# iden3/circom

Measured on NVIDIA B200. Metric: witnesses/s, higher is better.
Workload: dtype u256 (8x u32 limbs, Montgomery)

## Files before the change

circom_b200/csrc/capi.cu:

```cuda
#include <cuda_runtime.h>
#include <dlfcn.h>
#include <emmintrin.h>
#include <nccl.h>

#include <cstdio>
#include <cstdlib>
#include <algorithm>
#include <chrono>
#include <condition_variable>
#include <cstring>
#include <functional>
#include <map>
#include <memory>
#include <mutex>
#include <thread>
#include <stdexcept>
#include <string>
#include <vector>

#include "../../include/circom_b200.h"
#include "kernels.cuh"
#include "tape_calls.h"
#include "tape.h"
#include "hostpack.h"
// ... 195 lines not shown
        out = it->second;
        return CW_OK;
    }
    const Tape &t = c->tape;
    DevTape d;
    int rc;
    if ((rc = upload(&d.ops, t.ops.data(), t.ops.size() * 4))) return rc;
    if ((rc = upload(&d.items, t.items.data(), t.items.size() * 4))) return rc;
    {
        std::vector<uint32_t> heads(t.n_items() * 4);
        for (size_t k = 0; k < t.n_items(); ++k) memcpy(&heads[k * 4], &t.ops[(size_t)t.items[k] * 4], 16);
        if ((rc = upload(&d.heads, heads.data(), heads.size() * 4))) return rc;
    }
    if ((rc = upload(&d.level_start, t.level_start.data(), t.level_start.size() * 4))) return rc;
    {
        std::vector<uint32_t> info(t.n_levels(), 0);
        for (size_t l = 0; l < t.n_levels(); ++l) {
            bool tail = true;
            for (uint32_t k = t.level_start[l + 1]; k-- > t.level_start[l];) {
                const uint32_t opc = t.ops[(size_t)t.items[k] * 4] & 0xFFu;
                const bool single = t.items[k + 1] - t.items[k] == 1;
                const bool is_call = opc == 45u && single;
                if (opc == 45u && !(single && tail)) return fail(CW_ESTATE, "internal: a call is not at the end of its level");
                if (is_call) ++info[l];
                else tail = false;
                for (uint32_t w = t.items[k]; w < t.items[k + 1]; ++w) {
                    const uint32_t o = t.ops[(size_t)w * 4] & 0xFFu;
                    if (o == 28u || o == 5u) {
                        if (!single) return fail(CW_ESTATE, "internal: a fused work item contains INV / POW");
                        info[l] |= 0x80000000u;
                        d.has_slow = true;
                    }
                }
            }
        }
        if ((rc = upload(&d.level_info, info.data(), info.size() * 4))) return rc;
    }
    if ((rc = upload(&d.consts, t.consts.data(), t.consts.size() * 32))) return rc;
    if ((rc = upload(&d.input_slot, t.input_slot.data(), t.input_slot.size() * 4))) return rc;
    if ((rc = upload(&d.fn_code, t.fn_code.data(), t.fn_code.size() * 4))) return rc;
    if ((rc = upload(&d.fn_info, t.fn_info.data(), t.fn_info.size() * 4))) return rc;
    if ((rc = upload(&d.call_tab, t.call_tab.data(), t.call_tab.size() * 4))) return rc;
    if ((rc = upload(&d.wloc, t.witness_slot.data(), t.witness_slot.size() * 4))) return rc;
    if ((rc = upload(&d.pk_bit, L.bit_loc.data(), L.bit_loc.size() * 4))) return rc;
    if ((rc = upload(&d.pk_u64, L.u64_loc.data(), L.u64_loc.size() * 4))) return rc;
    if ((rc = upload(&d.pk_full, L.full_loc.data(), L.full_loc.size() * 4))) return rc;
    c->dev[device] = d;
    out = d;
    return CW_OK;
}

template <int PR, bool CALLS, bool BP, int BT, bool FU>
static void launch_tape_k(const TapeDev &tp, cw_batch *b, u32 tiles, u32 th) {
    tape_exec_kernel<PR, CALLS, BP, BT, FU><<<tiles, th, 0, b->stream>>>(tp, b->slots, b->plane, b->bt_log2, b->first_assert_d,
                                                                         b->err_d, b->batch);
}
template <int PR>
static void launch_tape(const TapeDev &tp, cw_batch *b, u32 tiles, u32 th, bool calls, bool bp, bool fused) {
    if (calls) {
        launch_tape_calls(PR, tp, b->slots, b->plane, b->bt_log2, b->first_assert_d, b->err_d, b->batch, tiles, th, bp, fused,
                          b->stream);
    } else if (fused) {
        if (b->bt_log2 == 5) launch_tape_k<PR, false, true, 5, true>(tp, b, tiles, th);
        else launch_tape_k<PR, false, true, -1, true>(tp, b, tiles, th);
    } else if (bp) {
        if (b->bt_log2 == 0) launch_tape_k<PR, false, true, 0, false>(tp, b, tiles, th);
        else if (b->bt_log2 == 5) launch_tape_k<PR, false, true, 5, false>(tp, b, tiles, th);
        else launch_tape_k<PR, false, true, -1, false>(tp, b, tiles, th);
    } else {
        if (b->bt_log2 == 0) launch_tape_k<PR, false, false, 0, false>(tp, b, tiles, th);
        else launch_tape_k<PR, false, false, -1, false>(tp, b, tiles, th);
    }
}

extern "C" {

int cw_version(void) { return 100; }
const char *cw_last_error(void) { return g_err.c_str(); }
int cw_device_count(void) {
    int n = 0;
    if (cudaGetDeviceCount(&n) != cudaSuccess) {
        cudaGetLastError();
        return 0;
    }
    return n;
}

int cw_circuit_load_mem(const void *data, size_t len, uint32_t flags, cw_circuit **out) {
    if (!data || !out) return fail(CW_EINVAL, "null argument");
    cw_circuit *c = new cw_circuit();
    try {
        lower_circuit((const uint8_t *)data, len, flags, c->tape);
    } catch (const std::exception &e) {
        delete c;
        return fail(CW_EFORMAT, e.what());
    }
    *out = c;
    return CW_OK;
}

int cw_circuit_load(const char *path, uint32_t flags, cw_circuit **out) {
    if (!path || !out) return fail(CW_EINVAL, "null argument");
    FILE *f = fopen(path, "rb");
    if (!f) return fail(CW_EIO, std::string("cannot open ") + path);
    fseek(f, 0, SEEK_END);
    long sz = ftell(f);
    fseek(f, 0, SEEK_SET);
    std::vector<uint8_t> buf(sz);
// ... 1518 lines not shown
```

circom_b200/csrc/flatten.cpp:

```cpp
#include <algorithm>
#include <bitset>
#include <cstdio>
#include <cstring>
#include <functional>
#include <stdexcept>
#include <unordered_map>

#include "../../include/circom_b200.h"
#include "tape.h"

namespace cw {

uint64_t fnv1a(const char *s, size_t n) {
    uint64_t h = 0xCBF29CE484222325ULL;
    for (size_t i = 0; i < n; ++i) {
        h ^= (uint64_t)(int64_t)(signed char)s[i];
        h *= 0x100000001B3ULL;
    }
    return h;
}

namespace {

enum { K_NONE = 0, K_OWN = 1, K_SUB = 2, K_CONST = 3, K_TMP = 4, K_ONE = 5 };
// ... 9 lines not shown
};
struct Tmpl {
    std::string name;
    uint32_t n_out, n_in, n_inter, n_tmp, n_own;
    std::vector<uint32_t> subs;
    std::vector<IrOp> ops;
    std::vector<uint32_t> lc_len;
    std::vector<Term> terms;
    std::vector<uint8_t> tmp_zero_only;
    uint64_t total_signals = 0, total_components = 0;
};

inline int rk(uint64_t r) { return (int)(r >> 56); }
inline uint32_t rsub(uint64_t r) { return (uint32_t)((r >> 32) & 0xFFFFFF); }
inline uint32_t ridx(uint64_t r) { return (uint32_t)r; }

struct Reader {
    const uint8_t *p, *end;
    template <class T>
    T get() {
        if (p + sizeof(T) > end) throw std::runtime_error("cb2c: truncated");
        T v;
        memcpy(&v, p, sizeof(T));
        p += sizeof(T);
        return v;
    }
    const uint8_t *bytes(size_t n) {
        if (n > (size_t)(end - p)) throw std::runtime_error("cb2c: truncated");
        const uint8_t *r = p;
        p += n;
        return r;
    }
    size_t left() const { return (size_t)(end - p); }
    void expect(uint64_t count, uint64_t bytes_each) const {
        if (count * bytes_each > left()) throw std::runtime_error("cb2c: truncated (count exceeds the file)");
    }
    std::string str() {
        uint32_t n = get<uint32_t>();
        const uint8_t *b = bytes((size_t)(((uint64_t)n + 3) & ~3ull));
        return std::string((const char *)b, n);
    }
};

struct Val {
    uint32_t slot[3] = {NO_SLOT, NO_SLOT, NO_SLOT};
    int32_t cid = -1;
    uint16_t bits = 256;
    uint8_t org_op = 0;
    int32_t org_a = -1, org_b = -1;
    int32_t fld_src = -1, bf_src = -1;
    uint16_t fld_k = 0, fld_m = 0, bf_lo = 0, bf_len = 0;
};

enum { DOP_BITS = 29, DOP_ASSERT_BOOL = 30, DOP_MULSMALL = 31, DOP_BITSIP = 32, DOP_ASSERT_FITS = 33 };
inline bool c_is_immediate(uint32_t opcode) {
    return opcode == CW_OP_ASSERT || opcode == CW_OP_ASSERT_EQ || opcode == DOP_BITS || opcode == DOP_ASSERT_BOOL ||
           opcode == DOP_BITSIP || opcode == DOP_ASSERT_FITS;
}
inline bool is_assert_op(uint32_t opcode) {
    return opcode == CW_OP_ASSERT || opcode == CW_OP_ASSERT_EQ || opcode == DOP_ASSERT_BOOL || opcode == DOP_ASSERT_FITS;
}

inline size_t n_live_ops(const std::vector<uint8_t> &live, uint32_t n_pre, size_t n_prov) {
    size_t n = 0;
    for (size_t i = 0; i < n_prov; ++i) n += live[n_pre + i];
    return n;
}
inline int subtree_need(uint32_t i, const std::vector<uint32_t> &kid_a, const std::vector<uint32_t> &kid_b) {
    const uint32_t a = kid_a[i], b = kid_b[i];
    if (a == NO_SLOT && b == NO_SLOT) return 1;
    if (a == NO_SLOT) return subtree_need(b, kid_a, kid_b);
    if (b == NO_SLOT) return subtree_need(a, kid_a, kid_b);
    const int na = subtree_need(a, kid_a, kid_b), nb = subtree_need(b, kid_a, kid_b);
    return std::max(std::max(na, nb), std::min(na, nb) + 1);
}

static uint32_t coalesce_function_copies(uint32_t *code, uint32_t n_instr, uint32_t n_regs, const std::vector<uint32_t> &fn_params) {
    constexpr uint32_t MAXR = 192;
    if (n_regs > MAXR || n_instr < 2) return n_instr;
    using Set = std::bitset<MAXR>;
    enum { JMP = 40, JZ = 41, RET = 42, LOADX = 43, STOREX = 44, CALLF = 45, COPY = 24 };
    auto is_reg = [&](uint32_t o) { return !(o & 0xC0000000u) && o < n_regs; };
    Set pinned;
    std::vector<uint8_t> target(n_instr + 1, 0);
    for (uint32_t i = 0; i < n_instr; ++i) {
        const uint32_t *w = &code[5 * (size_t)i];
        uint32_t lo = 0, hi = 0;
        if (w[0] == LOADX) { lo = w[2] & 0x3FFFFFFFu; hi = w[4] & 0x3FFFFFFFu; }
        else if (w[0] == STOREX) { lo = w[2] & 0x3FFFFFFFu; hi = w[1] & 0x3FFFFFFFu; }
        else if (w[0] == RET && (w[3] & 0x3FFFFFFFu) > 1) { lo = w[2]; hi = lo + (w[3] & 0x3FFFFFFFu); }
        else if (w[0] == CALLF) {
            for (uint32_t r = w[3]; r < w[3] + fn_params[w[2] & 0x3FFFFFFFu] && r < n_regs; ++r) pinned.set(r);
            if ((w[4] & 0x3FFFFFFFu) > 1) { lo = w[1]; hi = lo + (w[4] & 0x3FFFFFFFu); }
        }
        for (uint32_t r = lo; r < hi && r < n_regs; ++r) pinned.set(r);
        if (w[0] == JMP) target[std::min(w[2] & 0x3FFFFFFFu, n_instr)] = 1;
        if (w[0] == JZ) target[std::min(w[3] & 0x3FFFFFFFu, n_instr)] = 1;
    }
    std::vector<Set> use(n_instr), live_in(n_instr), live_out(n_instr);
    std::vector<int> def(n_instr, -1);
    auto add_use = [&](uint32_t i, uint32_t o) { if (is_reg(o) && !pinned.test(o)) use[i].set(o); };
    for (uint32_t i = 0; i < n_instr; ++i) {
        const uint32_t *w = &code[5 * (size_t)i];
        switch (w[0]) {
            case JMP: break;
            case JZ: add_use(i, w[2]); break;
            case RET: if ((w[3] & 0x3FFFFFFFu) <= 1) add_use(i, w[2]); break;
// ... 1149 lines not shown
            std::unordered_map<int32_t, uint32_t> entry_of_value;
            for (uint64_t i = 0; i < W; ++i) entry_of_value.emplace(sig_vid[T.witness2signal[i]], (uint32_t)i);
            std::unordered_map<std::string, uint32_t> const_at;
            auto log_const = [&](const U256 &v) {
                std::string key((const char *)v.v, 32);
                auto it = const_at.find(key);
                if (it != const_at.end()) return it->second;
                T.log_consts.push_back(v);
                return const_at.emplace(std::move(key), (uint32_t)T.log_consts.size() - 1).first->second;
            };
            for (const PendingLog &pl : pending_logs) {
                Tape::LogArg a;
                a.kind = pl.kind;
                a.last = pl.last ? 1 : 0;
                a.idx = (uint32_t)pl.idx;
                if (pl.kind == 2) a.idx = log_const(ir_consts[pl.idx]);
                if (pl.kind == 1) {
                    const int32_t v = sig_vid[pl.idx];
                    auto it = entry_of_value.find(v);
                    if (it != entry_of_value.end()) a.idx = it->second;
                    else if (vals[v].cid >= 0) { a.kind = 2; a.idx = log_const(ir_consts[vals[v].cid]); }
                    else throw std::runtime_error("lowering: log() of a signal whose value is not part of the witness");
                }
                T.log_args.push_back(a);
            }
        }
        std::vector<int64_t> claimed;
        std::vector<uint32_t> wsrc(W);
        auto grow = [&]() { claimed.resize(n_pre + pops.size() / 4, -1); };
        grow();
        for (uint64_t i = 0; i < W; ++i) {
            int32_t v = sig_vid[T.witness2signal[i]];
            uint32_t src;
            if (vals[v].cid >= 0) src = emit(CW_OP_COPY, const_operand(vals[v].cid, FC));
            else src = need(v, FC);
            grow();
            if (claimed[src] >= 0) {
                src = emit(CW_OP_COPY, src);
                grow();
            }
            claimed[src] = (int64_t)i;
            wsrc[i] = src;
            uint32_t wb = vbits(v);
            T.wit_bits.push_back((uint16_t)std::min<uint32_t>(wb, 256));
            if (wb <= 1) { T.pk_bit_wire.push_back((uint32_t)i); T.wit_class.push_back(0); }
            else if (wb <= 64) { T.pk_u64_wire.push_back((uint32_t)i); T.wit_class.push_back(1); }
            else { T.pk_full_wire.push_back((uint32_t)i); T.wit_class.push_back(2); }
        }
        size_t n_prov = pops.size() / 4;
        std::vector<uint16_t> slot_bits(n_pre + n_prov, 256);
        for (const Val &v : vals)
            if (v.cid < 0 && v.slot[FC] != NO_SLOT && v.slot[FC] < slot_bits.size())
                slot_bits[v.slot[FC]] = std::min<uint16_t>(slot_bits[v.slot[FC]], v.bits);
        for (uint64_t i = 0; i < W; ++i) {
            uint32_t wb = vbits(sig_vid[T.witness2signal[i]]);
            slot_bits[wsrc[i]] = std::min<uint16_t>(slot_bits[wsrc[i]], (uint16_t)wb);
        }
        std::vector<uint8_t> live(n_pre + n_prov, 0);
        for (uint64_t i = 0; i < W; ++i) live[wsrc[i]] = 1;
        for (size_t i = n_prov; i-- > 0;) {
            uint32_t *o = &pops[i * 4];
            bool is_assert = is_assert_op(o[0]);
            if (!is_assert && !live[n_pre + i]) continue;
            live[n_pre + i] = 1;
            if (o[0] == 45) {
                uint32_t n = pcalls[o[1] + 1];
                for (uint32_t k = 0; k < n; ++k) {
                    uint32_t a = pcalls[o[1] + 2 + k];
                    if (!(a & OPERAND_CONST)) live[a] = 1;
                }
                continue;
            }
            for (int k = 1; k <= 3; ++k) {
                if (k == 3 && c_is_immediate(o[0])) break;
                if (o[k] != NO_SLOT && !(o[k] & OPERAND_CONST)) live[o[k]] = 1;
            }
        }
        constexpr uint32_t FUSE_MAX = 24;
        std::vector<uint8_t> fusedf(n_prov, 0);
        std::vector<uint32_t> kid_a(n_prov, NO_SLOT), kid_b(n_prov, NO_SLOT);
        {
            std::vector<uint32_t> uses(n_pre + n_prov, 0), cons(n_pre + n_prov, NO_SLOT);
            std::vector<uint8_t> cons_pos(n_pre + n_prov, 0);
            for (size_t i = 0; i < n_prov; ++i) {
                if (!live[n_pre + i]) continue;
                const uint32_t *o = &pops[i * 4];
                if (o[0] == 45) {
                    uint32_t n = pcalls[o[1] + 1];
                    for (uint32_t k = 0; k < n; ++k) {
                        uint32_t x = pcalls[o[1] + 2 + k];
                        if (!(x & OPERAND_CONST)) uses[x] += 2;
                    }
                    continue;
                }
                for (int k = 1; k <= 3; ++k) {
                    if (k == 3 && c_is_immediate(o[0])) break;
                    if (o[k] == NO_SLOT || (o[k] & OPERAND_CONST)) continue;
                    ++uses[o[k]];
                    cons[o[k]] = (uint32_t)i;
                    cons_pos[o[k]] = (uint8_t)k;
                }
            }
            std::vector<uint8_t> need(n_prov, 1);
            std::vector<uint32_t> gsize(n_prov, 1);
            const bool fuse_on = (flags & CW_FLAG_FUSE) && !(flags & CW_FLAG_NO_PEEPHOLE) && pcalls.empty();
            auto candidate = [&](uint32_t slot, size_t reader, int pos) -> bool {
// ... 395 lines not shown
        }

    }
};

}

void lower_circuit(const uint8_t *data, size_t len, uint32_t flags, Tape &out) {
    Lowerer L(out, flags);
    L.parse(data, len);
    L.lower();
}

}

namespace cw {
namespace {
struct BlobW {
    std::vector<uint8_t> &o;
    void raw(const void *p, size_t n) { o.insert(o.end(), (const uint8_t *)p, (const uint8_t *)p + n); }
    template <class T> void pod(const T &v) { raw(&v, sizeof(T)); }
    template <class T> void vec(const std::vector<T> &v) {
        pod<uint64_t>(v.size());
        if (!v.empty()) raw(v.data(), v.size() * sizeof(T));
    }
    void str(const std::string &s) {
        pod<uint64_t>(s.size());
        raw(s.data(), s.size());
    }
};
struct BlobR {
    const uint8_t *p, *end;
    void raw(void *d, size_t n) {
        if (n > (size_t)(end - p)) throw std::runtime_error("lowered-circuit blob: truncated");
        memcpy(d, p, n);
        p += n;
    }
    template <class T> void pod(T &v) { raw(&v, sizeof(T)); }
    template <class T> void vec(std::vector<T> &v) {
        uint64_t n;
        pod(n);
        if (n > (uint64_t)(end - p) / sizeof(T)) throw std::runtime_error("lowered-circuit blob: bad length");
        v.resize(n);
        if (n) raw(v.data(), n * sizeof(T));
    }
    void str(std::string &s) {
        uint64_t n;
        pod(n);
        if (n > (uint64_t)(end - p)) throw std::runtime_error("lowered-circuit blob: bad length");
        s.assign((const char *)p, n);
        p += n;
    }
};
constexpr uint32_t BLOB_VERSION = 6;
}

void serialize_tape(const Tape &t, std::vector<uint8_t> &out) {
    BlobW w{out};
    w.raw("CB2T", 4);
    w.pod<uint32_t>(BLOB_VERSION);
    w.pod<int32_t>(t.F.prime_id);
    w.pod(t.flags);
    const uint64_t nums[] = {t.n_signals, t.n_witness, t.n_inputs, t.n_outputs, t.n_components, t.n_ir_ops, t.n_mul_ops,
                             t.n_conv_ops, t.max_level_width, t.n_asserts, t.slot_census[0], t.slot_census[1],
                             t.slot_census[2], t.slot_census[3], t.n_slot_operands, t.n_values, t.n_resident, t.n_pre,
                             t.n_slots, t.n_bitwords, t.n_stored};
    w.pod<uint64_t>(sizeof(nums) / 8);
    w.raw(nums, sizeof(nums));
    w.vec(t.ops); w.vec(t.items); w.vec(t.level_start); w.vec(t.consts); w.vec(t.dat_consts); w.vec(t.witness_slot); w.vec(t.input_slot);
    w.vec(t.pk_bit_wire); w.vec(t.pk_u64_wire); w.vec(t.pk_full_wire); w.vec(t.wit_class); w.vec(t.wit_bits);
    w.vec(t.fn_code); w.vec(t.fn_info); w.vec(t.call_tab); w.vec(t.witness2signal);
    w.pod<uint64_t>(t.inputs.size());
    for (const InputInfo &in : t.inputs) {
        w.str(in.name);
        w.pod(in.hash); w.pod(in.signal_id); w.pod(in.size);
    }
    w.vec(t.hashmap);
    const R1csData &r = t.r1cs;
    w.pod<int32_t>(r.prime_id);
    w.pod(r.n_wires); w.pod(r.n_constraints);
    w.vec(r.row_ptr); w.vec(r.col); w.vec(r.coef); w.vec(r.dict);
    w.pod(r.n_pub_out); w.pod(r.n_pub_in); w.pod(r.n_prv_in);
}

void deserialize_tape(const uint8_t *data, size_t len, Tape &t) {
    BlobR r{data, data + len};
    char magic[4];
    r.raw(magic, 4);
    uint32_t ver;
    r.pod(ver);
    if (memcmp(magic, "CB2T", 4) || ver != BLOB_VERSION) throw std::runtime_error("lowered-circuit blob: bad magic / version");
    int32_t prime;
    r.pod(prime);
    if (prime < 0 || prime >= CW_N_PRIMES) throw std::runtime_error("lowered-circuit blob: unknown prime");
    t.F = make_field(prime);
    r.pod(t.flags);
    uint64_t n_nums;
    r.pod(n_nums);
    uint64_t nums[21];
    if (n_nums != 21) throw std::runtime_error("lowered-circuit blob: layout mismatch");
    r.raw(nums, sizeof(nums));
    t.n_signals = nums[0]; t.n_witness = nums[1]; t.n_inputs = nums[2]; t.n_outputs = nums[3]; t.n_components = nums[4];
    t.n_ir_ops = nums[5]; t.n_mul_ops = nums[6]; t.n_conv_ops = nums[7]; t.max_level_width = nums[8]; t.n_asserts = nums[9];
    for (int k = 0; k < 4; ++k) t.slot_census[k] = nums[10 + k];
    t.n_slot_operands = nums[14]; t.n_values = nums[15]; t.n_resident = (uint32_t)nums[16]; t.n_pre = (uint32_t)nums[17];
    t.n_slots = (uint32_t)nums[18]; t.n_bitwords = (uint32_t)nums[19]; t.n_stored = nums[20];
    r.vec(t.ops); r.vec(t.items); r.vec(t.level_start); r.vec(t.consts); r.vec(t.dat_consts); r.vec(t.witness_slot); r.vec(t.input_slot);
// ... 28 lines not shown
```

circom_b200/csrc/fr_device.cuh:

```cuda
#pragma once
#include <stddef.h>
#include <stdint.h>

#if defined(__CUDACC__)
#define CW_HD __host__ __device__ __forceinline__
#else
#define CW_HD inline
#endif

namespace cw {

typedef uint32_t u32;
typedef uint64_t u64;

struct FrParams {
    u32 q[8];
    u32 half[8];
    u32 r1[8];
    u32 r2[8];
    u32 qm2[8];
    u32 np32;
    u32 qbits;
    u32 top_mask;
    u32 pad;
// ... 518 lines not shown
            u32 t[8];
            u256_shl(t, quo, bit);
            u256_sub(rem, a, t);
            return true;
        }
    }
    u32 lza = u256_clz(a);
    u32 n[8], q[8], r[8];
    if (lza == 256) {
        u256_set_u32(quo, 0);
        u256_set_u32(rem, 0);
        return true;
    }
    u256_shl(n, a, lza);
    u256_set_u32(q, 0);
    u256_set_u32(r, 0);
    int steps = 256 - (int)lza;
#if defined(__CUDA_ARCH__)
#pragma unroll 1
#endif
    for (int i = 0; i < steps; ++i) {
        u32 carry = n[7] >> 31;
#pragma unroll
        for (int j = 7; j > 0; --j) n[j] = (n[j] << 1) | (n[j - 1] >> 31);
        n[0] <<= 1;
        const u32 rtop = r[7] >> 31;
#pragma unroll
        for (int j = 7; j > 0; --j) r[j] = (r[j] << 1) | (r[j - 1] >> 31);
        r[0] = (r[0] << 1) | carry;
        u32 t[8];
        u32 br = u256_sub(t, r, b);
#pragma unroll
        for (int j = 7; j > 0; --j) q[j] = (q[j] << 1) | (q[j - 1] >> 31);
        q[0] <<= 1;
        if (rtop || !br) {
            u256_set(r, t);
            q[0] |= 1;
        }
    }
    u256_set(quo, q);
    u256_set(rem, r);
    return true;
}

enum {
    OP_MUL = 1, OP_ADD = 3, OP_SUB = 4, OP_POW = 5, OP_IDIV = 6, OP_MOD = 7, OP_SHL = 8, OP_SHR = 9,
    OP_LEQ = 10, OP_GEQ = 11, OP_LT = 12, OP_GT = 13, OP_EQ = 14, OP_NEQ = 15, OP_LOR = 16, OP_LAND = 17,
    OP_LNOT = 18, OP_BOR = 19, OP_BAND = 20, OP_BXOR = 21, OP_BNOT = 22, OP_NEG = 23, OP_COPY = 24,
    OP_SELECT = 25, OP_ASSERT = 26, OP_ASSERT_EQ = 27, OP_INV = 28,
    OP_BITS = 29,
    OP_ASSERT_BOOL = 30,
    OP_MULSMALL = 31,
    OP_BITSIP = 32,
    OP_ASSERT_FITS = 33
};

CW_HD void u256_mul_lo(u32 *r, const u32 *a, const u32 *b) {
    u32 t[8];
#pragma unroll
    for (int i = 0; i < 8; ++i) t[i] = 0;
#pragma unroll
    for (int i = 0; i < 8; ++i) {
        u64 c = 0;
#pragma unroll
        for (int j = 0; j + i < 8; ++j) {
            c += (u64)a[j] * b[i] + t[i + j];
            t[i + j] = (u32)c;
            c >>= 32;
        }
    }
    u256_set(r, t);
}
CW_HD void u256_bits(u32 *r, const u32 *a, u32 imm) {
    u32 k = imm & 0xFFFFu, m = (imm >> 16) & 0xFFu;
    u32 t[8];
    u256_shr(t, a, k);
#pragma unroll
    for (int i = 0; i < 8; ++i) {
        int lo = i * 32;
        u32 mask = (int)m >= lo + 32 ? 0xFFFFFFFFu : ((int)m <= lo ? 0u : ((1u << (m - lo)) - 1u));
        r[i] = t[i] & mask;
    }
}

CW_HD void u256_bits_in_place(u32 *r, const u32 *a, u32 imm) {
    u32 lo = imm & 0xFFu, len = imm >> 8, hi = lo + len;
#pragma unroll
    for (int i = 0; i < 8; ++i) {
        u32 b0 = 32u * i, b1 = b0 + 32u;
        u32 m = 0;
        if (hi > b0 && lo < b1) {
            u32 from = lo > b0 ? lo - b0 : 0u, to = hi < b1 ? hi - b0 : 32u;
            u32 w = to - from;
            m = (w >= 32u ? 0xFFFFFFFFu : ((1u << w) - 1u)) << from;
        }
        r[i] = a[i] & m;
    }
}
CW_HD u32 u256_bitlen(const u32 *a) {
    u32 n = 0;
#pragma unroll
    for (int i = 0; i < 8; ++i) {
        if (a[i]) {
            u32 x = a[i], c = 0;
            while (x) { x >>= 1; ++c; }
            n = 32u * i + c;
        }
    }
    return n;
}

template <bool SLOW>
CW_HD void fr_exec_t(u32 opcode, u32 *r, const u32 *a, const u32 *b, u32 imm, const FrParams &P, int &err) {
    switch (opcode) {
        case OP_BITSIP: u256_bits_in_place(r, a, imm); break;
        case OP_BITS: u256_bits(r, a, imm); break;
        case OP_MULSMALL: u256_mul_lo(r, a, b); break;
        case OP_MUL: fr_mont_mul(r, a, b, P); break;
        case OP_ADD: fr_add(r, a, b, P); break;
        case OP_SUB: fr_sub(r, a, b, P); break;
        case OP_NEG: fr_neg(r, a, P); break;
        case OP_INV: if (SLOW) fr_inv_mont(r, a, P); break;
        case OP_POW: if (SLOW) fr_pow_mont(r, a, b, P); break;
        case OP_IDIV: { u32 rem[8]; if (!u256_divmod(r, rem, a, b)) err = 1; break; }
        case OP_MOD: { u32 quo[8]; if (!u256_divmod(quo, r, a, b)) err = 1; break; }
        case OP_SHL: fr_shl(r, a, b, P); break;
        case OP_SHR: fr_shr(r, a, b, P); break;
        case OP_LT: u256_set_u32(r, fr_lt(a, b, P)); break;
        case OP_GT: u256_set_u32(r, fr_lt(b, a, P)); break;
        case OP_LEQ: u256_set_u32(r, !fr_lt(b, a, P)); break;
        case OP_GEQ: u256_set_u32(r, !fr_lt(a, b, P)); break;
        case OP_EQ: u256_set_u32(r, u256_eq(a, b)); break;
        case OP_NEQ: u256_set_u32(r, !u256_eq(a, b)); break;
        case OP_LOR: u256_set_u32(r, !u256_is_zero(a) || !u256_is_zero(b)); break;
        case OP_LAND: u256_set_u32(r, !u256_is_zero(a) && !u256_is_zero(b)); break;
        case OP_LNOT: u256_set_u32(r, u256_is_zero(a)); break;
        case OP_BOR:
#pragma unroll
            for (int i = 0; i < 8; ++i) r[i] = a[i] | b[i];
            fr_mask_wrap(r, P);
            break;
        case OP_BAND:
#pragma unroll
            for (int i = 0; i < 8; ++i) r[i] = a[i] & b[i];
            fr_mask_wrap(r, P);
            break;
        case OP_BXOR:
#pragma unroll
            for (int i = 0; i < 8; ++i) r[i] = a[i] ^ b[i];
            fr_mask_wrap(r, P);
            break;
        case OP_BNOT:
#pragma unroll
            for (int i = 0; i < 8; ++i) r[i] = ~a[i];
            fr_mask_wrap(r, P);
            break;
        case OP_COPY: u256_set(r, a); break;
        default: u256_set_u32(r, 0); break;
    }
}
CW_HD void fr_exec(u32 opcode, u32 *r, const u32 *a, const u32 *b, u32 imm, const FrParams &P, int &err) {
    fr_exec_t<true>(opcode, r, a, b, imm, P, err);
}

CW_HD void fr_apply_canonical(u32 op, u32 *r, const u32 *a, const u32 *b, const u32 *c, const FrParams &P, int &err) {
    if (op == OP_MUL) {
        if (u256_bitlen(a) + u256_bitlen(b) < P.qbits) {
            u256_mul_lo(r, a, b);
        } else {
            u32 am[8];
            fr_to_mont(am, a, P);
            fr_mont_mul(r, am, b, P);
        }
    } else if (op == 2 ) {
        u32 bm[8], im[8];
        fr_to_mont(bm, b, P);
        fr_inv_mont(im, bm, P);
        fr_mont_mul(r, im, a, P);
    } else if (op == OP_POW) {
        u32 am[8], rm[8];
        fr_to_mont(am, a, P);
        fr_pow_mont(rm, am, b, P);
        fr_from_mont(r, rm, P);
    } else if (op == OP_SELECT) {
        bool t = !u256_is_zero(c);
        for (int k = 0; k < 8; ++k) r[k] = t ? a[k] : b[k];
    } else {
        fr_exec(op, r, a, b, 0, P, err);
    }
}

enum { FOP_JMP = 40, FOP_JZ = 41, FOP_RET = 42, FOP_LOADX = 43, FOP_STOREX = 44, OP_CALL = 45 };
enum { VM_MAX_REGS = 192, VM_MAX_STEPS = 1 << 22, VM_MAX_DEPTH = 8 };
struct FnInfo {
    u32 code_off, n_instr, n_regs, n_params;
};
CW_HD FnInfo vm_fn(const u32 *fn_info, u32 f) {
    FnInfo fi;
    fi.code_off = fn_info[4 * (size_t)f];
    fi.n_instr = fn_info[4 * (size_t)f + 1];
    fi.n_regs = fn_info[4 * (size_t)f + 2];
    fi.n_params = fn_info[4 * (size_t)f + 3];
    return fi;
}
struct VmFrame {
    u32 fn, pc, base, dst, want;
};

CW_HD void vm_operand(u32 *v, u32 o, const u32 *regs, const u32 *consts32) {
    if (o & 0x80000000u) {
        const u32 *p = consts32 + 8 * (size_t)(o & 0x3FFFFFFFu);
        for (int k = 0; k < 8; ++k) v[k] = p[k];
// ... 290 lines not shown
```

circom_b200/csrc/kernels.cuh:

```cuda
#pragma once
#include <cuda_runtime.h>
#include <stdint.h>

#include "fr_device.cuh"
#include "r1cs_small.h"

namespace cw {

constexpr int N_PRIMES_DEV = 8;
__constant__ FrParams c_fr[N_PRIMES_DEV];
#define CW_FR(PRIME, rt) c_fr[(PRIME) >= 0 ? (PRIME) : (int)(rt)]

__device__ __forceinline__ void ldg256(u32 *v, const void *p) {
    asm volatile("ld.global.v8.b32 {%0,%1,%2,%3,%4,%5,%6,%7}, [%8];"
                 : "=r"(v[0]), "=r"(v[1]), "=r"(v[2]), "=r"(v[3]), "=r"(v[4]), "=r"(v[5]), "=r"(v[6]), "=r"(v[7])
                 : "l"(p)
                 : "memory");
}
__device__ __forceinline__ void ldg256_nc(u32 *v, const void *p) {
    asm("ld.global.nc.v8.b32 {%0,%1,%2,%3,%4,%5,%6,%7}, [%8];"
        : "=r"(v[0]), "=r"(v[1]), "=r"(v[2]), "=r"(v[3]), "=r"(v[4]), "=r"(v[5]), "=r"(v[6]), "=r"(v[7])
        : "l"(p));
}
__device__ __forceinline__ void stg256(void *p, const u32 *v) {
// ... 101 lines not shown

#endif

template <int PRIME, int TAG>
__device__ __noinline__ void exec_slow_op(u32 opcode, u32 *r, const u32 *a, const u32 *b, u32 prime_rt) {
    const FrParams &P = CW_FR(PRIME, prime_rt);
    if (opcode == OP_INV) fr_inv_mont(r, a, P);
    else fr_pow_mont(r, a, b, P);
}

template <int PRIME, bool BP, int TAG>
__device__ __noinline__ void exec_call(const TapeDev &tp, u32 call_off, uint4 *base, const u32 *plane_base,
                                       u32 bt_log2, u32 li, u32 *r, int *err) {
    const FrParams &P = CW_FR(PRIME, tp.prime);
    const u32 *ct = tp.call_tab + call_off;
    const u32 f = __ldg(&ct[0]), n_args = __ldg(&ct[1]);
    FnInfo fi;
    fi.code_off = __ldg(&tp.fn_info[4 * f]);
    fi.n_instr = __ldg(&tp.fn_info[4 * f + 1]);
    fi.n_regs = __ldg(&tp.fn_info[4 * f + 2]);
    fi.n_params = __ldg(&tp.fn_info[4 * f + 3]);
    u32 regs[VM_MAX_REGS * 8];
    for (u32 k = 0; k < n_args; ++k) {
        u32 v[8];
        load_operand<BP>(v, __ldg(&ct[2 + k]), base, plane_base, tp.consts, bt_log2, li);
        for (int j = 0; j < 8; ++j) regs[8 * k + j] = v[j];
    }
    int e = 0;
    u32 ret_base, ret_cnt;
    const bool narrow = !tp.vm_wide && vm_run_narrow(tp.fn_code, tp.fn_info, f, regs, reinterpret_cast<const u32 *>(tp.consts), r,
                                                     e, ret_base, ret_cnt);
    if (!narrow) {
        for (u32 k = 0; k < fi.n_regs * 8; ++k) regs[k] = 0;
        for (u32 k = 0; k < n_args; ++k) {
            u32 v[8];
            load_operand<BP>(v, __ldg(&ct[2 + k]), base, plane_base, tp.consts, bt_log2, li);
            for (int j = 0; j < 8; ++j) regs[8 * k + j] = v[j];
        }
        e = 0;
        vm_run(tp.fn_code, tp.fn_info, f, regs, reinterpret_cast<const u32 *>(tp.consts), r, P, e, ret_base, ret_cnt);
    }
    const u32 n_extra = __ldg(&ct[2 + n_args]);
    for (u32 k = 0; k < n_extra; ++k) {
        const u32 d = __ldg(&ct[3 + n_args + k]);
        if (d == 0xFFFFFFFFu) continue;
        if (k + 1 >= ret_cnt) { e = 2; continue; }
        u32 v[8];
        vm_result(v, regs, ret_base + k + 1, narrow);
        store_slot(v, base, d, bt_log2, li);
    }
    *err = e;
}

#ifndef CW_TAPE_LB
#define CW_TAPE_LB 512
#endif
#ifndef CW_TAPE_MINB
#define CW_TAPE_MINB 2
#endif
template <int PRIME, bool HAS_CALLS, bool BP, int BT, bool FUSED>
__global__ void __launch_bounds__(CW_TAPE_LB, CW_TAPE_MINB)
    tape_exec_kernel(TapeDev tp, uint4 *__restrict__ slots, u32 *__restrict__ plane, u32 bt_log2_arg,
                     u32 *__restrict__ first_assert, int *__restrict__ err, u32 batch) {
    const FrParams &P = CW_FR(PRIME, tp.prime);
    const u32 bt_log2 = BT >= 0 ? (u32)BT : bt_log2_arg;
    constexpr bool COOP = BT == 0 && !HAS_CALLS && !BP;
    const u32 tile = blockIdx.x;
    const u32 bt_mask = (1u << bt_log2) - 1;
    uint4 *base = slots + (((size_t)tile * tp.n_slots) << (bt_log2 + 1));
    u32 *plane_base = BP ? plane + (((size_t)tile * tp.n_bitwords) << bt_log2) : nullptr;
    u32 lb = tp.level_start[0];
    u32 le = tp.n_levels ? tp.level_start[1] : lb;
    uint4 pre = make_uint4(0, 0, 0, 0);
    u32 pre_g0 = 0, pre_g1 = 0;
    if (threadIdx.x < ((le - lb) << bt_log2)) {
        if (FUSED) {
            pre_g0 = __ldg(&tp.items[lb + (threadIdx.x >> bt_log2)]);
            pre_g1 = __ldg(&tp.items[lb + (threadIdx.x >> bt_log2) + 1]);
            pre = __ldg(&tp.heads[lb + (threadIdx.x >> bt_log2)]);
        } else pre = __ldg(&tp.ops[lb + (threadIdx.x >> bt_log2)]);
    }
    for (u32 l = 0; l < tp.n_levels; ++l) {
        const u32 info = (HAS_CALLS || tp.has_slow) ? __ldg(&tp.level_info[l]) : 0u;
        const u32 n_calls = HAS_CALLS ? (info & 0x7FFFFFFFu) : 0u;
        const u32 n = (le - lb - n_calls) << bt_log2;
        const u32 le_next = (l + 1 < tp.n_levels) ? tp.level_start[l + 2] : le;
        for (u32 w0 = COOP ? (threadIdx.x & ~31u) : threadIdx.x; w0 < n; w0 += blockDim.x) {
            const u32 w = COOP ? w0 + (threadIdx.x & 31u) : w0;
            u32 run_dst = 0, run_n = 0, run_bits = 0;
            if (!COOP || w < n) {
            const u32 li = w & bt_mask;
            const u32 inst = (tile << bt_log2) + li;
            const bool first = w == threadIdx.x;
            u32 g0 = lb + (w >> bt_log2), g1 = g0 + 1u;
            if (FUSED) {
                g0 = first ? pre_g0 : __ldg(&tp.items[lb + (w >> bt_log2)]);
                g1 = first ? pre_g1 : __ldg(&tp.items[lb + (w >> bt_log2) + 1]);
            }
            u32 acc0[8], acc1[8];
            uint4 nxt = pre;
            if (!first) {
                if (FUSED) nxt = __ldg(&tp.heads[lb + (w >> bt_log2)]);
                else nxt = __ldg(&tp.ops[g0]);
            }
            for (u32 k = g0; k < g1; ++k) {
            const uint4 opw = nxt;
            bool has_value = true;
            if (FUSED && k + 1 < g1) nxt = __ldg(&tp.ops[k + 1]);
            const u32 opcode = opw.x & 0xFFu, dst = opw.x >> 8;
            u32 r[8];
            if (opcode == OP_BITS && ((opw.w >> 16) & 0xFFu) <= 32u && !(opw.y & (OPD_CONST | OPD_BIT | OPD_ACC))) {
                const u32 kk = opw.w & 0xFFFFu, m = (opw.w >> 16) & 0xFFu, run = (opw.w >> 24) + 1u;
                const u32 wd = kk >> 5, sh = kk & 31u;
                const bool two = sh + m + run - 1u > 32u && wd < 7u;
                u32 lo, hi = 0;
                {
                    const u32 *words = reinterpret_cast<const u32 *>(base);
                    const size_t src = (size_t)(opw.y & OPD_SLOT) << (bt_log2 + 1);
                    const u32 w1 = wd + 1u;
                    lo = words[((src + ((size_t)(wd >> 2) << bt_log2) + li) << 2) + (wd & 3u)];
                    if (two) hi = words[((src + ((size_t)(w1 >> 2) << bt_log2) + li) << 2) + (w1 & 3u)];
                }
                const unsigned long long window = (((unsigned long long)hi << 32) | lo) >> sh;
#pragma unroll
                for (int i = 1; i < 8; ++i) r[i] = 0;
                if (run > 1u) {
                    if (BP && tp.n_bitwords) {
                        plane_base[((size_t)dst << bt_log2) + li] =
                            (u32)window & (run >= 32u ? 0xFFFFFFFFu : ((1u << run) - 1u));
                    } else if (COOP) {
                        run_dst = dst;
                        run_n = run;
                        run_bits = (u32)window;
                    } else {
                        for (u32 j = 0; j < run; ++j) {
                            r[0] = (u32)(window >> j) & 1u;
                            store_slot(r, base, dst + j, bt_log2, li);
                        }
                    }
                    has_value = false;
                } else r[0] = (u32)window & (m >= 32u ? 0xFFFFFFFFu : ((1u << m) - 1u));
            } else {
                u32 a[8], b[8];
                if (FUSED && !(opw.y & OPD_CONST) && (opw.y & OPD_ACC)) {
#pragma unroll
                    for (int i = 0; i < 8; ++i) a[i] = (opw.y & 1u) ? acc1[i] : acc0[i];
                } else load_operand<BP>(a, opw.y, base, plane_base, tp.consts, bt_log2, li);
                if (FUSED && !(opw.z & OPD_CONST) && (opw.z & OPD_ACC)) {
#pragma unroll
                    for (int i = 0; i < 8; ++i) b[i] = (opw.z & 1u) ? acc1[i] : acc0[i];
                } else load_operand<BP>(b, opw.z, base, plane_base, tp.consts, bt_log2, li);
                if (opcode == OP_SELECT) {
                    u32 c[8];
                    load_operand<BP>(c, opw.w, base, plane_base, tp.consts, bt_log2, li);
                    bool t = !u256_is_zero(c);
#pragma unroll
                    for (int i = 0; i < 8; ++i) r[i] = t ? a[i] : b[i];
                } else if (opcode == OP_ASSERT_EQ || opcode == OP_ASSERT || opcode == OP_ASSERT_BOOL ||
                           opcode == OP_ASSERT_FITS) {
                    bool ok = opcode == OP_ASSERT_EQ     ? u256_eq(a, b)
                              : opcode == OP_ASSERT      ? !u256_is_zero(a)
                              : opcode == OP_ASSERT_BOOL ? (u256_is_zero(a) || u256_eq(a, b))
                                                         : (u256_bitlen_dev(a) <= b[0]);
                    if (!ok && inst < batch) atomicMin(&first_assert[inst], opw.w);
                    has_value = false;
                } else if (opcode == OP_INV || opcode == OP_POW) {
                    has_value = false;
                } else {
                    int e = 0;
                    fr_exec_t<false>(opcode, r, a, b, opw.w, P, e);
                    if (e && inst < batch) err[inst] = 1;
                }
            }
            if (has_value) {
                if (FUSED && dst >= DST_ACC_DEV) {
#pragma unroll
                    for (int i = 0; i < 8; ++i) {
                        if (dst & 1u) acc1[i] = r[i];
                        else acc0[i] = r[i];
                    }
                } else store_slot(r, base, dst, bt_log2, li);
            }
            }
            }
            if (COOP) {
                unsigned pending = __ballot_sync(0xFFFFFFFFu, run_n != 0u);
                const u32 lane = threadIdx.x & 31u;
                while (pending) {
                    const int src = __ffs(pending) - 1;
                    pending &= pending - 1u;
                    const u32 d = __shfl_sync(0xFFFFFFFFu, run_dst, src);
                    const u32 cnt = __shfl_sync(0xFFFFFFFFu, run_n, src);
                    const u32 bits = __shfl_sync(0xFFFFFFFFu, run_bits, src);
                    if (lane < cnt) {
                        u32 r[8] = {(bits >> lane) & 1u, 0u, 0u, 0u, 0u, 0u, 0u, 0u};
                        stg256(base + ((size_t)(d + lane) << 1), r);
                    }
                }
            }
        }
        if (info >> 31) {
            for (u32 w = threadIdx.x; w < n; w += blockDim.x) {
                const u32 li = w & bt_mask;
                const uint4 opw = __ldg(&tp.ops[FUSED ? __ldg(&tp.items[lb + (w >> bt_log2)]) : lb + (w >> bt_log2)]);
                const u32 opcode = opw.x & 0xFFu;
                if (opcode != OP_INV && opcode != OP_POW) continue;
                u32 a[8], b[8], r[8];
                load_operand<BP>(a, opw.y, base, plane_base, tp.consts, bt_log2, li);
                load_operand<BP>(b, opw.z, base, plane_base, tp.consts, bt_log2, li);
                exec_slow_op<PRIME, (HAS_CALLS ? 64 : 0) + (BP ? 32 : 0) + (BT + 1) * 2 + (FUSED ? 1 : 0)>(opcode, r, a, b, tp.prime);
                store_slot(r, base, opw.x >> 8, bt_log2, li);
            }
        }
        if (HAS_CALLS && n_calls) {
            const u32 cb = le - n_calls;
            for (u32 w = threadIdx.x; w < (n_calls << bt_log2); w += blockDim.x) {
                const u32 li = w & bt_mask;
                const u32 inst = (tile << bt_log2) + li;
                const uint4 opw = __ldg(&tp.ops[FUSED ? __ldg(&tp.items[cb + (w >> bt_log2)]) : cb + (w >> bt_log2)]);
                u32 r[8];
                int e = 0;
                exec_call<PRIME, BP, BT * 2 + (FUSED ? 1 : 0)>(tp, opw.y, base, plane_base, bt_log2, li, r, &e);
                if (e && inst < batch) err[inst] = 1;
                store_slot(r, base, opw.x >> 8, bt_log2, li);
            }
        }
        if (threadIdx.x < ((le_next - le) << bt_log2)) {
            if (FUSED) {
                pre_g0 = __ldg(&tp.items[le + (threadIdx.x >> bt_log2)]);
                pre_g1 = __ldg(&tp.items[le + (threadIdx.x >> bt_log2) + 1]);
                pre = __ldg(&tp.heads[le + (threadIdx.x >> bt_log2)]);
            } else pre = __ldg(&tp.ops[le + (threadIdx.x >> bt_log2)]);
        }
        lb = le;
// ... 423 lines not shown
```

circom_b200/native.py:

```python
from __future__ import annotations

import ctypes
import os
from ctypes import POINTER, c_char_p, c_float, c_int, c_int32, c_int64, c_size_t, c_uint8, c_uint32, c_uint64, c_void_p

from . import build as _build

CW_OK, CW_EINVAL, CW_EIO, CW_EFORMAT, CW_ECUDA, CW_ENOTFOUND, CW_ESTATE, CW_ENODEV = 0, -1, -2, -3, -4, -5, -6, -7
CW_FLAG_NO_ASSERTS, CW_FLAG_HOST_ONLY, CW_FLAG_O0, CW_FLAG_NO_PEEPHOLE, CW_FLAG_BITPLANE, CW_FLAG_REUSE = 1, 2, 4, 8, 16, 32
CW_FLAG_COMPACT = CW_FLAG_BITPLANE | CW_FLAG_REUSE
CW_FLAG_FUSE = 64


class CwError(RuntimeError):
    def __init__(self, code: int, msg: str):
        super().__init__("circom_b200 error %d: %s" % (code, msg))
        self.code = code


class CwStats(ctypes.Structure):
    _fields_ = [(n, c_uint64) for n in (
        "n_signals", "n_witness", "n_inputs", "n_outputs", "n_components", "n_constants", "n_ir_ops",
        "n_tape_ops", "n_slots", "n_levels", "n_constraints", "n_nnz", "n_mul_ops", "n_conv_ops",
        "max_level_width", "n_slot_operands", "n_bitwords", "n_resident_slots", "n_items", "n_stored", "n_values")]

    def as_dict(self):
        return {n: int(getattr(self, n)) for n, _ in self._fields_}


def _load() -> ctypes.CDLL:
    path = os.environ.get("CW_LIB_PATH") or _build.LIB
    if not os.path.exists(path):
        _build.build()
    lib = ctypes.CDLL(path)
    P = c_void_p
    sig = {
        "cw_version": (c_int, []),
        "cw_last_error": (c_char_p, []),
        "cw_device_count": (c_int, []),
        "cw_circuit_load": (c_int, [c_char_p, c_uint32, POINTER(P)]),
        "cw_circuit_load_mem": (c_int, [c_void_p, c_size_t, c_uint32, POINTER(P)]),
        "cw_circuit_destroy": (None, [P]),
        "cw_circuit_stats": (c_int, [P, POINTER(CwStats)]),
        "cw_circuit_prime": (c_int, [P, POINTER(c_int), POINTER(c_uint64)]),
        "cw_get_main_input_signal_start": (c_uint32, [P]),
        "cw_get_main_input_signal_no": (c_uint32, [P]),
        "cw_get_total_signal_no": (c_uint32, [P]),
        "cw_get_number_of_components": (c_uint32, [P]),
        "cw_get_size_of_input_hashmap": (c_uint32, [P]),
        "cw_get_size_of_witness": (c_uint32, [P]),
        "cw_get_size_of_constants": (c_uint32, [P]),
        "cw_fnv1a": (c_uint64, [c_char_p]),
        "cw_get_input_signal_size": (c_int, [P, c_uint64, POINTER(c_uint64)]),
        "cw_get_input_signal_id": (c_int, [P, c_uint64, POINTER(c_uint64)]),
        "cw_circuit_tape": (c_int, [P, c_void_p, c_void_p, c_void_p]),
        "cw_circuit_tape_items": (c_int, [P, c_void_p]),
        "cw_circuit_slot_census": (c_int, [P, POINTER(c_uint64)]),
        "cw_circuit_witness2signal": (c_int, [P, c_void_p]),
        "cw_circuit_write_dat": (c_int, [P, c_char_p]),
        "cw_circuit_write_sym": (c_int, [P, c_char_p]),
        "cw_circuit_functions": (c_int, [P, POINTER(c_uint32), POINTER(c_uint32)]),
        "cw_batch_create": (c_int, [P, c_uint32, c_int, POINTER(P)]),
        "cw_batch_destroy": (None, [P]),
        "cw_batch_set_input": (c_int, [P, c_uint32, c_uint64, c_uint32, POINTER(c_uint64)]),
# ... 67 lines not shown
```

include/circom_b200.h:

```cpp
#ifndef CIRCOM_B200_H
#define CIRCOM_B200_H

#include <stddef.h>
#include <stdint.h>

#ifdef __cplusplus
extern "C" {
#endif

#define CW_OK 0
#define CW_EINVAL (-1)
#define CW_EIO (-2)
#define CW_EFORMAT (-3)
#define CW_ECUDA (-4)
#define CW_ENOTFOUND (-5)
#define CW_ESTATE (-6)
#define CW_ENODEV (-7)

#define CW_PRIME_BN128 0
#define CW_PRIME_BLS12381 1
#define CW_PRIME_GRUMPKIN 2
#define CW_PRIME_PALLAS 3
#define CW_PRIME_VESTA 4
#define CW_PRIME_SECQ256R1 5
#define CW_PRIME_BLS12377 6
#define CW_PRIME_GOLDILOCKS 7

#define CW_FLAG_NO_ASSERTS 1u
#define CW_FLAG_HOST_ONLY 2u
#define CW_FLAG_NO_PEEPHOLE 8u
#define CW_FLAG_BITPLANE 16u
#define CW_FLAG_REUSE 32u
#define CW_FLAG_FUSE 64u
#define CW_FLAG_COMPACT (CW_FLAG_BITPLANE | CW_FLAG_REUSE)
#define CW_FLAG_O0 4u

enum cw_op {
    CW_OP_NOP = 0, CW_OP_MUL = 1, CW_OP_DIV = 2, CW_OP_ADD = 3, CW_OP_SUB = 4, CW_OP_POW = 5,
    CW_OP_IDIV = 6, CW_OP_MOD = 7, CW_OP_SHL = 8, CW_OP_SHR = 9, CW_OP_LEQ = 10, CW_OP_GEQ = 11,
    CW_OP_LT = 12, CW_OP_GT = 13, CW_OP_EQ = 14, CW_OP_NEQ = 15, CW_OP_LOR = 16, CW_OP_LAND = 17,
    CW_OP_LNOT = 18, CW_OP_BOR = 19, CW_OP_BAND = 20, CW_OP_BXOR = 21, CW_OP_BNOT = 22,
    CW_OP_NEG = 23, CW_OP_COPY = 24, CW_OP_SELECT = 25, CW_OP_ASSERT = 26, CW_OP_ASSERT_EQ = 27,
    CW_OP_INV = 28
};

typedef struct cw_circuit cw_circuit;
typedef struct cw_batch cw_batch;
typedef struct cw_r1cs cw_r1cs;

typedef struct cw_stats {
    uint64_t n_signals;
    uint64_t n_witness;
    uint64_t n_inputs;
    uint64_t n_outputs;
    uint64_t n_components;
    uint64_t n_constants;
    uint64_t n_ir_ops;
    uint64_t n_tape_ops;
    uint64_t n_slots;
    uint64_t n_levels;
    uint64_t n_constraints;
    uint64_t n_nnz;
    uint64_t n_mul_ops;
    uint64_t n_conv_ops;
    uint64_t max_level_width;
    uint64_t n_slot_operands;
    uint64_t n_bitwords;
    uint64_t n_resident_slots;
    uint64_t n_items;
    uint64_t n_stored;
    uint64_t n_values;
} cw_stats;

int cw_version(void);
const char *cw_last_error(void);
int cw_device_count(void);

int cw_circuit_load(const char *cb2c_path, uint32_t flags, cw_circuit **out);
int cw_circuit_load_mem(const void *data, size_t len, uint32_t flags, cw_circuit **out);
void cw_circuit_destroy(cw_circuit *c);
int cw_circuit_stats(const cw_circuit *c, cw_stats *out);
int cw_circuit_prime(const cw_circuit *c, int *prime_id, uint64_t q[4]);
uint32_t cw_get_main_input_signal_start(const cw_circuit *c);
uint32_t cw_get_main_input_signal_no(const cw_circuit *c);
uint32_t cw_get_total_signal_no(const cw_circuit *c);
uint32_t cw_get_number_of_components(const cw_circuit *c);
// ... 88 lines not shown
```

Baseline: 198,600.

## Add bit-width-typed opcodes and move fused accumulators to shared memory

The flattener now rewrites adds, small multiplies and constant shifts into specialised opcodes when the slot bit-width analysis shows no modular reduction is needed. Examples are a non-reducing add, a 128-bit add, truncated 4- or 6-limb multiplies and immediate shifts, all meant to cut per-op arithmetic in the tape interpreter. On the host path each typed result is checked against the general op. Separately, the fused kernel's two 8-limb accumulators move from registers (acc0/acc1) into dynamic shared memory, which should lower register pressure at the cost of shared-memory traffic and some occupancy limit. The typed opcodes are on by default unless the new NO_TYPED flag is set.

```diff
diff --git a/circom_b200/csrc/capi.cu b/circom_b200/csrc/capi.cu
--- a/circom_b200/csrc/capi.cu
+++ b/circom_b200/csrc/capi.cu
@@ -271,8 +271,9 @@
 
 template <int PR, bool CALLS, bool BP, int BT, bool FU>
 static void launch_tape_k(const TapeDev &tp, cw_batch *b, u32 tiles, u32 th) {
-    tape_exec_kernel<PR, CALLS, BP, BT, FU><<<tiles, th, 0, b->stream>>>(tp, b->slots, b->plane, b->bt_log2, b->first_assert_d,
-                                                                         b->err_d, b->batch);
+    static_assert(tape_acc_smem(CW_TAPE_LB) <= 48u * 1024u, "the accumulators of the widest CTA need an opt-in shared-memory size");
+    tape_exec_kernel<PR, CALLS, BP, BT, FU><<<tiles, th, FU ? tape_acc_smem(th) : 0u, b->stream>>>(
+        tp, b->slots, b->plane, b->bt_log2, b->first_assert_d, b->err_d, b->batch);
 }
 template <int PR>
 static void launch_tape(const TapeDev &tp, cw_batch *b, u32 tiles, u32 th, bool calls, bool bp, bool fused) {
diff --git a/circom_b200/csrc/flatten.cpp b/circom_b200/csrc/flatten.cpp
--- a/circom_b200/csrc/flatten.cpp
+++ b/circom_b200/csrc/flatten.cpp
@@ -85,7 +85,8 @@
     uint16_t fld_k = 0, fld_m = 0, bf_lo = 0, bf_len = 0;
 };
 
-enum { DOP_BITS = 29, DOP_ASSERT_BOOL = 30, DOP_MULSMALL = 31, DOP_BITSIP = 32, DOP_ASSERT_FITS = 33 };
+enum { DOP_BITS = 29, DOP_ASSERT_BOOL = 30, DOP_MULSMALL = 31, DOP_BITSIP = 32, DOP_ASSERT_FITS = 33,
+       DOP_ADD_NR = 34, DOP_ADD128 = 35, DOP_MULSMALL128 = 36, DOP_MULSMALL192 = 37, DOP_SHRI = 38, DOP_SHLI = 39 };
 inline bool c_is_immediate(uint32_t opcode) {
     return opcode == CW_OP_ASSERT || opcode == CW_OP_ASSERT_EQ || opcode == DOP_BITS || opcode == DOP_ASSERT_BOOL ||
            opcode == DOP_BITSIP || opcode == DOP_ASSERT_FITS;
@@ -1341,6 +1342,22 @@
         for (const Val &v : vals)
             if (v.cid < 0 && v.slot[FC] != NO_SLOT && v.slot[FC] < slot_bits.size())
                 slot_bits[v.slot[FC]] = std::min<uint16_t>(slot_bits[v.slot[FC]], v.bits);
+        if (!(flags & CW_FLAG_NO_TYPED)) {
+            const uint32_t lim = qb() - 1;
+            auto const_amount = [&](uint32_t o) {
+                if (o == NO_SLOT || !(o & OPERAND_CONST)) return false;
+                const U256 &c = consts[o & ~OPERAND_CONST];
+                return !(c.v[1] | c.v[2] | c.v[3]) && c.v[0] < qb();
+            };
+            for (size_t i = 0; i < n_prov; ++i) {
+                uint32_t *o = &pops[i * 4];
+                const uint32_t bits = slot_bits[n_pre + i];
+                if (o[0] == CW_OP_ADD && bits <= lim) o[0] = bits <= 128 ? DOP_ADD128 : DOP_ADD_NR;
+                else if (o[0] == DOP_MULSMALL && bits <= 192) o[0] = bits <= 128 ? DOP_MULSMALL128 : DOP_MULSMALL192;
+                else if (o[0] == CW_OP_SHR && const_amount(o[2])) o[0] = DOP_SHRI;
+                else if (o[0] == CW_OP_SHL && bits <= lim && const_amount(o[2])) o[0] = DOP_SHLI;
+            }
+        }
         for (uint64_t i = 0; i < W; ++i) {
             uint32_t wb = vbits(sig_vid[T.witness2signal[i]]);
             slot_bits[wsrc[i]] = std::min<uint16_t>(slot_bits[wsrc[i]], (uint16_t)wb);
@@ -1842,7 +1859,7 @@
         p += n;
     }
 };
-constexpr uint32_t BLOB_VERSION = 6;
+constexpr uint32_t BLOB_VERSION = 7;
 }
 
 void serialize_tape(const Tape &t, std::vector<uint8_t> &out) {
diff --git a/circom_b200/csrc/fr_device.cuh b/circom_b200/csrc/fr_device.cuh
--- a/circom_b200/csrc/fr_device.cuh
+++ b/circom_b200/csrc/fr_device.cuh
@@ -594,7 +594,13 @@
     OP_ASSERT_BOOL = 30,
     OP_MULSMALL = 31,
     OP_BITSIP = 32,
-    OP_ASSERT_FITS = 33
+    OP_ASSERT_FITS = 33,
+    OP_ADD_NR = 34,
+    OP_ADD128 = 35,
+    OP_MULSMALL128 = 36,
+    OP_MULSMALL192 = 37,
+    OP_SHRI = 38,
+    OP_SHLI = 39
 };
 
 CW_HD void u256_mul_lo(u32 *r, const u32 *a, const u32 *b) {
@@ -612,6 +618,34 @@
         }
     }
     u256_set(r, t);
+}
+template <int K>
+CW_HD void u256_mul_lo_k(u32 *r, const u32 *a, const u32 *b) {
+    u32 t[8];
+#pragma unroll
+    for (int i = 0; i < 8; ++i) t[i] = 0;
+#pragma unroll
+    for (int i = 0; i < K; ++i) {
+        u64 c = 0;
+#pragma unroll
+        for (int j = 0; j + i < K; ++j) {
+            c += (u64)a[j] * b[i] + t[i + j];
+            t[i + j] = (u32)c;
+            c >>= 32;
+        }
+    }
+    u256_set(r, t);
+}
+CW_HD void u256_add_lo4(u32 *r, const u32 *a, const u32 *b) {
+    u64 c = 0;
+#pragma unroll
+    for (int i = 0; i < 4; ++i) {
+        c += (u64)a[i] + b[i];
+        r[i] = (u32)c;
+        c >>= 32;
+    }
+#pragma unroll
+    for (int i = 4; i < 8; ++i) r[i] = 0;
 }
 CW_HD void u256_bits(u32 *r, const u32 *a, u32 imm) {
     u32 k = imm & 0xFFFFu, m = (imm >> 16) & 0xFFu;
@@ -652,14 +686,29 @@
     return n;
 }
 
+CW_HD bool fr_typed_holds(u32 opcode, const u32 *r, const u32 *a, const u32 *b, const FrParams &P) {
+    u32 g[8];
+    if (opcode == OP_ADD_NR || opcode == OP_ADD128) fr_add(g, a, b, P);
+    else if (opcode == OP_MULSMALL128 || opcode == OP_MULSMALL192) u256_mul_lo(g, a, b);
+    else if (opcode == OP_SHRI) fr_shr(g, a, b, P);
+    else fr_shl(g, a, b, P);
+    return u256_eq(g, r) && !u256_geq(r, P.q);
+}
+
 template <bool SLOW>
 CW_HD void fr_exec_t(u32 opcode, u32 *r, const u32 *a, const u32 *b, u32 imm, const FrParams &P, int &err) {
     switch (opcode) {
         case OP_BITSIP: u256_bits_in_place(r, a, imm); break;
         case OP_BITS: u256_bits(r, a, imm); break;
         case OP_MULSMALL: u256_mul_lo(r, a, b); break;
+        case OP_MULSMALL128: u256_mul_lo_k<4>(r, a, b); break;
+        case OP_MULSMALL192: u256_mul_lo_k<6>(r, a, b); break;
         case OP_MUL: fr_mont_mul(r, a, b, P); break;
         case OP_ADD: fr_add(r, a, b, P); break;
+        case OP_ADD_NR: u256_add(r, a, b); break;
+        case OP_ADD128: u256_add_lo4(r, a, b); break;
+        case OP_SHRI: u256_shr(r, a, b[0]); break;
+        case OP_SHLI: u256_shl(r, a, b[0]); break;
         case OP_SUB: fr_sub(r, a, b, P); break;
         case OP_NEG: fr_neg(r, a, P); break;
         case OP_INV: if (SLOW) fr_inv_mont(r, a, P); break;
@@ -700,6 +749,9 @@
         case OP_COPY: u256_set(r, a); break;
         default: u256_set_u32(r, 0); break;
     }
+#if !defined(__CUDA_ARCH__)
+    if (opcode >= OP_ADD_NR && opcode <= OP_SHLI && !fr_typed_holds(opcode, r, a, b, P)) err = 1;
+#endif
 }
 CW_HD void fr_exec(u32 opcode, u32 *r, const u32 *a, const u32 *b, u32 imm, const FrParams &P, int &err) {
     fr_exec_t<true>(opcode, r, a, b, imm, P, err);
diff --git a/circom_b200/csrc/kernels.cuh b/circom_b200/csrc/kernels.cuh
--- a/circom_b200/csrc/kernels.cuh
+++ b/circom_b200/csrc/kernels.cuh
@@ -177,6 +177,17 @@
     *err = e;
 }
 
+__host__ __device__ constexpr unsigned tape_acc_smem(unsigned threads) { return 4u * threads * (unsigned)sizeof(uint4); }
+__device__ __forceinline__ void load_acc(u32 *v, const uint4 *s_acc, u32 k) {
+    const uint4 lo = s_acc[(2u * k) * blockDim.x + threadIdx.x], hi = s_acc[(2u * k + 1u) * blockDim.x + threadIdx.x];
+    v[0] = lo.x; v[1] = lo.y; v[2] = lo.z; v[3] = lo.w;
+    v[4] = hi.x; v[5] = hi.y; v[6] = hi.z; v[7] = hi.w;
+}
+__device__ __forceinline__ void store_acc(const u32 *v, uint4 *s_acc, u32 k) {
+    s_acc[(2u * k) * blockDim.x + threadIdx.x] = make_uint4(v[0], v[1], v[2], v[3]);
+    s_acc[(2u * k + 1u) * blockDim.x + threadIdx.x] = make_uint4(v[4], v[5], v[6], v[7]);
+}
+
 #ifndef CW_TAPE_LB
 #define CW_TAPE_LB 512
 #endif
@@ -194,6 +205,7 @@
     const u32 bt_mask = (1u << bt_log2) - 1;
     uint4 *base = slots + (((size_t)tile * tp.n_slots) << (bt_log2 + 1));
     u32 *plane_base = BP ? plane + (((size_t)tile * tp.n_bitwords) << bt_log2) : nullptr;
+    extern __shared__ uint4 s_acc[];
     u32 lb = tp.level_start[0];
     u32 le = tp.n_levels ? tp.level_start[1] : lb;
     uint4 pre = make_uint4(0, 0, 0, 0);
@@ -222,7 +234,6 @@
                 g0 = first ? pre_g0 : __ldg(&tp.items[lb + (w >> bt_log2)]);
                 g1 = first ? pre_g1 : __ldg(&tp.items[lb + (w >> bt_log2) + 1]);
             }
-            u32 acc0[8], acc1[8];
             uint4 nxt = pre;
             if (!first) {
                 if (FUSED) nxt = __ldg(&tp.heads[lb + (w >> bt_log2)]);
@@ -267,14 +278,10 @@
                 } else r[0] = (u32)window & (m >= 32u ? 0xFFFFFFFFu : ((1u << m) - 1u));
             } else {
                 u32 a[8], b[8];
-                if (FUSED && !(opw.y & OPD_CONST) && (opw.y & OPD_ACC)) {
-#pragma unroll
-                    for (int i = 0; i < 8; ++i) a[i] = (opw.y & 1u) ? acc1[i] : acc0[i];
-                } else load_operand<BP>(a, opw.y, base, plane_base, tp.consts, bt_log2, li);
-                if (FUSED && !(opw.z & OPD_CONST) && (opw.z & OPD_ACC)) {
-#pragma unroll
-                    for (int i = 0; i < 8; ++i) b[i] = (opw.z & 1u) ? acc1[i] : acc0[i];
-                } else load_operand<BP>(b, opw.z, base, plane_base, tp.consts, bt_log2, li);
+                if (FUSED && !(opw.y & OPD_CONST) && (opw.y & OPD_ACC)) load_acc(a, s_acc, opw.y & 1u);
+                else load_operand<BP>(a, opw.y, base, plane_base, tp.consts, bt_log2, li);
+                if (FUSED && !(opw.z & OPD_CONST) && (opw.z & OPD_ACC)) load_acc(b, s_acc, opw.z & 1u);
+                else load_operand<BP>(b, opw.z, base, plane_base, tp.consts, bt_log2, li);
                 if (opcode == OP_SELECT) {
                     u32 c[8];
                     load_operand<BP>(c, opw.w, base, plane_base, tp.consts, bt_log2, li);
@@ -298,13 +305,8 @@
                 }
             }
             if (has_value) {
-                if (FUSED && dst >= DST_ACC_DEV) {
-#pragma unroll
-                    for (int i = 0; i < 8; ++i) {
-                        if (dst & 1u) acc1[i] = r[i];
-                        else acc0[i] = r[i];
-                    }
-                } else store_slot(r, base, dst, bt_log2, li);
+                if (FUSED && dst >= DST_ACC_DEV) store_acc(r, s_acc, dst & 1u);
+                else store_slot(r, base, dst, bt_log2, li);
             }
             }
             }
diff --git a/circom_b200/native.py b/circom_b200/native.py
--- a/circom_b200/native.py
+++ b/circom_b200/native.py
@@ -10,6 +10,7 @@
 CW_FLAG_NO_ASSERTS, CW_FLAG_HOST_ONLY, CW_FLAG_O0, CW_FLAG_NO_PEEPHOLE, CW_FLAG_BITPLANE, CW_FLAG_REUSE = 1, 2, 4, 8, 16, 32
 CW_FLAG_COMPACT = CW_FLAG_BITPLANE | CW_FLAG_REUSE
 CW_FLAG_FUSE = 64
+CW_FLAG_NO_TYPED = 128
 
 
 class CwError(RuntimeError):
diff --git a/include/circom_b200.h b/include/circom_b200.h
--- a/include/circom_b200.h
+++ b/include/circom_b200.h
@@ -32,6 +32,7 @@
 #define CW_FLAG_BITPLANE 16u
 #define CW_FLAG_REUSE 32u
 #define CW_FLAG_FUSE 64u
+#define CW_FLAG_NO_TYPED 128u
 #define CW_FLAG_COMPACT (CW_FLAG_BITPLANE | CW_FLAG_REUSE)
 #define CW_FLAG_O0 4u
 
```

New measurement: 229,100, median of 6. +15.4%, better.
